# marvinli00/genie2

Measured on AMD Instinct MI355X. Metric: denoise-steps/sec (N=256, T=1000, batch=8), higher is better.
Workload: dtype f32 (pair-stack products as 3 f16 MFMAs on 2xf16-split operands, f32 accumulate); 1 GPU; unconditional N=256, T=1000, batch=8 per GPU, random-init base Denoiser (15.7M params), scale=0.6, reverse-loop steps 995..676; parallelism=replica per GPU x1, no data-path collective

## Files before the change

### genie2_amd/csrc/pair_hx_kernels.hip

```cpp
#include "hx_pair.h"


template <int NW>
__global__ __launch_bounds__(NW * 64, NW == 8 ? 1 : 2) void k_pair_transition_hx(
    float* __restrict__ z, const float* __restrict__ rmask, const unsigned char* __restrict__ wimg,
    const float* __restrict__ b1s, const float* __restrict__ b2s, int N, long long M, int n_hb, float sx, float c1, float c2, int rev) {
    extern __shared__ __attribute__((aligned(16))) unsigned char smb[];
    float* sb1 = reinterpret_cast<float*>(smb + 2 * HX_STAGE_BYTES);
    const int lane = threadIdx.x & 63, wave = UNI(threadIdx.x >> 6);
    const int h = lane >> 5, pl = lane & 31;
    const int n_wt = (int)((M + 31) / 32);
    const int n_tiles = (n_wt + NW - 1) / NW;
    const rsrc_t rw = hx_rsrc(wimg, (unsigned)(n_hb * HX_STAGE_BYTES));
    const rsrc_t rz = hx_rsrc(z, (unsigned)(M * 512));
    const rsrc_t rnull = hx_rsrc(z, 0u);
    const int lane16 = lane * 16;
    constexpr int PW = 32 / NW;
    auto issue = [&](int hb, int buf) {
#pragma unroll
        for (int q = 0; q < PW; ++q) {
            const int p = PW * wave + q;
            hx_dma(rw, smb + buf * HX_STAGE_BYTES + p * 1024, lane16, hb * HX_STAGE_BYTES + p * 1024);
        }
    };
// ... 334 lines not shown
    __syncthreads();
    int kc = 0;
    const int foff = (lane & 31) * CX_ROWB + (lane >> 5) * 16;
    for (int it = 0; it < total; ++it) {
        const bool last_chunk = kc == nk - 1;
        const int wn_next = last_chunk ? w + gridDim.x : w;
        const int kc_next = last_chunk ? 0 : kc + 1;
        if (it + 1 < total) gload(wn_next, kc_next);
        const unsigned char* sa = smb + (it & 1) * 4 * PLANE + foff;
        h8 ah[WT], al[WT], bh[WT], bl[WT];
#pragma unroll
        for (int m = 0; m < WT; ++m) {
            ah[m] = *reinterpret_cast<const h8*>(sa + (wm * WT + m) * 32 * CX_ROWB);
            al[m] = *reinterpret_cast<const h8*>(sa + PLANE + (wm * WT + m) * 32 * CX_ROWB);
        }
#pragma unroll
        for (int n = 0; n < WT; ++n) {
            bh[n] = *reinterpret_cast<const h8*>(sa + 2 * PLANE + (wn * WT + n) * 32 * CX_ROWB);
            bl[n] = *reinterpret_cast<const h8*>(sa + 3 * PLANE + (wn * WT + n) * 32 * CX_ROWB);
        }
#pragma unroll
        for (int m = 0; m < WT; ++m)
#pragma unroll
            for (int n = 0; n < WT; ++n) MFH3(ah[m], al[m], bh[n], bl[n], acc[m][n]);
        if (last_chunk) {
            int mi, i0, j0;
            decode(w, mi, i0, j0);
            if (mi < n_mat) {
                const int vst = ((4 * (lane >> 5)) * NP + (lane & 31)) * 4;
#pragma unroll
                for (int m = 0; m < WT; ++m)
#pragma unroll
                    for (int n = 0; n < WT; ++n) {
                        const int ib = i0 + (wm * WT + m) * 32, jb = j0 + (wn * WT + n) * 32;
                        if (ib < NP && jb < NP) {
                            const int sbase = ((mi * NP + ib) * NP + jb) * 4;
#pragma unroll
                            for (int r = 0; r < 16; ++r) {
                                const float v = acc[m][n][r] * cx;
                                hx_store(rx, v, vst, sbase + ((r & 3) + 8 * (r >> 2)) * NP * 4);
                            }
                        }
                        acc[m][n] = zero16();
                    }
            }
        }
        if (it + 1 < total) swrite((it + 1) & 1);
        __syncthreads();
        w = wn_next;
        kc = kc_next;
    }
}

#define CB_ROWB 80
#define CB_PLANE (256 * CB_ROWB)
__global__ __launch_bounds__(512, 1) void k_trimul_contract_hx_big(const unsigned* __restrict__ acm, const unsigned* __restrict__ bcm,
                                                                   float* __restrict__ xcm, int NP, int n_mat, unsigned cm_bytes, float cx, int rev) {
    extern __shared__ __attribute__((aligned(16))) unsigned char smb[];
    const int tid = threadIdx.x, lane = tid & 63;
    const int wave = UNI(tid >> 6);
    const int wm = wave >> 1, wn = wave & 1;
    const int nk = NP / 32;
    const rsrc_t ra = hx_rsrc(acm, cm_bytes), rb = hx_rsrc(bcm, cm_bytes), rx = hx_rsrc(xcm, cm_bytes);
    const int gq = tid >> 3, pc = tid & 7;
    const int lr = (gq & 0x38) | ((gq & 1) << 2) | ((gq >> 1) & 3);
    u32x4 rA[2][4], rB[2][4];
    auto mat_of = [&](int w) { return rev ? n_mat - 1 - w : w; };
    auto gload = [&](int w, int kc, auto set_tag) {
        constexpr int S = decltype(set_tag)::value;
        const int mbase = mat_of(w) * NP * NP * 4 + kc * 128;
#pragma unroll
        for (int u = 0; u < 4; ++u) {
            const int row = 64 * u + lr;
            const int vo = row < NP ? (row * NP * 4 + pc * 16) : 0x7FFFFFF0;
            rA[S][u] = __builtin_bit_cast(u32x4, __builtin_amdgcn_raw_buffer_load_b128(ra, vo, mbase, 0));
            rB[S][u] = __builtin_bit_cast(u32x4, __builtin_amdgcn_raw_buffer_load_b128(rb, vo, mbase, 0));
        }
    };
    auto swrite = [&](auto set_tag) {
        constexpr int S = decltype(set_tag)::value;
        unsigned char* sa = smb + lr * CB_ROWB + pc * 8;
#pragma unroll
        for (int u = 0; u < 4; ++u) {
            uint2 ahi, alo, bhi, blo;
            ahi.x = __builtin_amdgcn_perm(rA[S][u].y, rA[S][u].x, 0x05040100u); ahi.y = __builtin_amdgcn_perm(rA[S][u].w, rA[S][u].z, 0x05040100u);
            alo.x = __builtin_amdgcn_perm(rA[S][u].y, rA[S][u].x, 0x07060302u); alo.y = __builtin_amdgcn_perm(rA[S][u].w, rA[S][u].z, 0x07060302u);
            bhi.x = __builtin_amdgcn_perm(rB[S][u].y, rB[S][u].x, 0x05040100u); bhi.y = __builtin_amdgcn_perm(rB[S][u].w, rB[S][u].z, 0x05040100u);
            blo.x = __builtin_amdgcn_perm(rB[S][u].y, rB[S][u].x, 0x07060302u); blo.y = __builtin_amdgcn_perm(rB[S][u].w, rB[S][u].z, 0x07060302u);
            *reinterpret_cast<uint2*>(sa + 64 * u * CB_ROWB) = ahi;
            *reinterpret_cast<uint2*>(sa + CB_PLANE + 64 * u * CB_ROWB) = alo;
            *reinterpret_cast<uint2*>(sa + 2 * CB_PLANE + 64 * u * CB_ROWB) = bhi;
            *reinterpret_cast<uint2*>(sa + 3 * CB_PLANE + 64 * u * CB_ROWB) = blo;
        }
    };
    f32x16 acc[2][4];
#pragma unroll
    for (int m = 0; m < 2; ++m)
#pragma unroll
        for (int n = 0; n < 4; ++n) acc[m][n] = zero16();
    int w = blockIdx.x;
    if (w >= n_mat) return;
    const int my = (n_mat - 1 - w) / gridDim.x + 1;
    const int total = my * nk;
    int lw = w, lkc = 0, issued = 0;
    auto advance = [&]() { if (lkc == nk - 1) { lw += gridDim.x; lkc = 0; } else ++lkc; };
    gload(lw, lkc, std::integral_constant<int, 0>{}); advance(); ++issued;
    if (issued < total) { gload(lw, lkc, std::integral_constant<int, 1>{}); advance(); ++issued; }
    int kc = 0;
    const int foff = (lane & 31) * CB_ROWB + (lane >> 5) * 16;
    const bool wave_live = 64 * wm < NP && 128 * wn < NP;
    auto body = [&](int it, auto set_tag) {
        const bool last_chunk = kc == nk - 1;
        swrite(set_tag);
        __syncthreads();
        if (issued < total) { gload(lw, lkc, set_tag); advance(); ++issued; }
        if (wave_live) {
#pragma unroll
            for (int c = 0; c < 2; ++c) {
                const unsigned char* sa = smb + foff + c * 32;
                h8 ah[2], al[2], bh[4], bl[4];
#pragma unroll
                for (int m = 0; m < 2; ++m) {
                    ah[m] = *reinterpret_cast<const h8*>(sa + (wm * 2 + m) * 32 * CB_ROWB);
                    al[m] = *reinterpret_cast<const h8*>(sa + CB_PLANE + (wm * 2 + m) * 32 * CB_ROWB);
                }
#pragma unroll
                for (int n = 0; n < 4; ++n) {
                    bh[n] = *reinterpret_cast<const h8*>(sa + 2 * CB_PLANE + (wn * 4 + n) * 32 * CB_ROWB);
                    bl[n] = *reinterpret_cast<const h8*>(sa + 3 * CB_PLANE + (wn * 4 + n) * 32 * CB_ROWB);
                }
#pragma unroll
                for (int m = 0; m < 2; ++m)
#pragma unroll
                    for (int n = 0; n < 4; ++n) MFH3(ah[m], al[m], bh[n], bl[n], acc[m][n]);
            }
        }
        if (last_chunk) {
            const int mi = mat_of(w);
            const int vst = ((4 * (lane >> 5)) * NP + (lane & 31)) * 4;
#pragma unroll
            for (int m = 0; m < 2; ++m)
#pragma unroll
                for (int n = 0; n < 4; ++n) {
                    const int ib = (wm * 2 + m) * 32, jb = (wn * 4 + n) * 32;
                    if (ib < NP && jb < NP) {
                        const int sbase = ((mi * NP + ib) * NP + jb) * 4;
#pragma unroll
                        for (int r = 0; r < 16; ++r) {
                            const float v = acc[m][n][r] * cx;
#if HX_ABL & 512
                            if (r == 0)
#endif
                            hx_store(rx, v, vst, sbase + ((r & 3) + 8 * (r >> 2)) * NP * 4);
                        }
                    }
                    acc[m][n] = zero16();
                }
            w += gridDim.x;
            kc = 0;
        } else
            ++kc;
        __syncthreads();
    };
    for (int it = 0; it < total; it += 2) {
        body(it, std::integral_constant<int, 0>{});
        if (it + 1 < total) body(it + 1, std::integral_constant<int, 1>{});
    }
}

template <int NW>
__global__ __launch_bounds__(NW * 64, NW == 8 ? 1 : 2) void k_trimul_out_hx(
    float* __restrict__ z, const float* __restrict__ xcm, const unsigned char* __restrict__ wimg,
    const float* __restrict__ bgs, const float* __restrict__ bzs, int N, int NP, int n_wtiles, unsigned cm_bytes,
    unsigned z_bytes, float sx, float cg, float cz, int rev) {
    extern __shared__ __attribute__((aligned(16))) unsigned char smb[];
    const int lane = threadIdx.x & 63, wave = UNI(threadIdx.x >> 6);
    const int h = lane >> 5, pl = lane & 31;
    const int ntile = (N + 31) >> 5;
    const int n_tiles = (n_wtiles + NW - 1) / NW;
    const rsrc_t rw = hx_rsrc(wimg, 4 * HX_STAGE_BYTES);
    const rsrc_t rx = hx_rsrc(xcm, cm_bytes), rz = hx_rsrc(z, z_bytes);
    const int lane16 = lane * 16;
    constexpr int PW = 32 / NW;
    auto issue = [&](int s, int buf) {
#pragma unroll
        for (int q = 0; q < PW; ++q) {
            const int p = PW * wave + q;
            hx_dma(rw, smb + buf * HX_STAGE_BYTES + p * 1024, lane16, s * HX_STAGE_BYTES + p * 1024);
        }
    };
    unsigned char* zt = smb + 2 * HX_STAGE_BYTES + 2048 + wave * HX_ZT_BYTES;
    int tile = blockIdx.x;
    issue(0, 0);
    __syncthreads();
#pragma unroll 1
    for (; tile < n_tiles; tile += gridDim.x) {
        const int wt_raw = HX_PHYS(tile) * NW + wave;
        const bool act = wt_raw < n_wtiles;
        const int wt = act ? wt_raw : n_wtiles - 1;
        const int st = wt % ntile, i = (wt / ntile) % N, b = wt / (ntile * N);
        const int t0 = st * 32;
        const int nvalid = act ? min(32, N - t0) : 0;
        const int prow0 = (b * N + i) * N + t0;
        const bool more = tile + (int)gridDim.x < n_tiles;
        h8 zh[8], zl[8], xh[8], xl[8];
        {
            float4 raw[16], rawz[16];
            const int cs = NP * NP * 4;
            const int vx = (8 * h * NP * NP + pl) * 4;
            const int sxo = ((b * 128 * NP + i) * NP + t0) * 4;
#pragma unroll
            for (int kc = 0; kc < 8; ++kc) {
                raw[2 * kc].x = hx_load(rx, vx, sxo + (16 * kc + 0) * cs); raw[2 * kc].y = hx_load(rx, vx, sxo + (16 * kc + 1) * cs);
                raw[2 * kc].z = hx_load(rx, vx, sxo + (16 * kc + 2) * cs); raw[2 * kc].w = hx_load(rx, vx, sxo + (16 * kc + 3) * cs);
                raw[2 * kc + 1].x = hx_load(rx, vx, sxo + (16 * kc + 4) * cs); raw[2 * kc + 1].y = hx_load(rx, vx, sxo + (16 * kc + 5) * cs);
                raw[2 * kc + 1].z = hx_load(rx, vx, sxo + (16 * kc + 6) * cs); raw[2 * kc + 1].w = hx_load(rx, vx, sxo + (16 * kc + 7) * cs);
            }
            const int zsoff = prow0 * 512, znv = min(32, N - t0);
            hx_zt_dma(rz, zt, lane, zsoff, 512, znv, 0); hx_vm_done(); hx_zt_read(rawz, zt, pl, h, 0); hx_lds_done();
            hx_zt_dma(rz, zt, lane, zsoff, 512, znv, 1);
            hx_norm_split(xh, xl, raw, sx);
            hx_vm_done(); hx_zt_read(rawz, zt, pl, h, 1);
// ... 249 lines not shown
static int hx_nw() { return 8; }
static unsigned hx_grid(long long n_tiles, int nw, int cus) {
    const long long cap = (nw == 8 ? 1LL : 2LL) * cus;
    return (unsigned)(n_tiles < cap ? n_tiles : cap);
}

struct HxSlice { int b0, nb; hipStream_t st; int cus; unsigned launches; bool prof; };

static void pair_transition_slice(genie_ctx* h, HxSlice& v, const PairLayerW& w) {
    const int N = h->N;
    const long long M = (long long)v.nb * N * N;
    const long long n_wt = (M + 31) / 32;
    const int n_hb = h->d.pair_transition_n * 4;
    const HxTransW& x = w.hx_pt;
    hipLaunchKernelGGL(k_pair_transition_hx<8>, dim3(hx_grid((n_wt + 7) / 8, 8, v.cus)), dim3(512), HX_LDS_BYTES, v.st,
                       h->p + (size_t)v.b0 * N * N * 128, h->rmaskf + (size_t)v.b0 * N, x.img, x.b1s, x.b2s, N, M, n_hb, x.sx, x.c1, x.c2,
                       (int)(v.launches++ & 1));
}

struct HxTriGeom {
    int N, NP, ntile, nw, n_wt;
    unsigned *acm, *bcm; float* xcm; float* zs; const float* ms;
    unsigned cm_bytes, z_bytes;
};
static HxTriGeom tri_geom(genie_ctx* h, const HxSlice& v) {
    HxTriGeom g;
    g.N = h->N; g.NP = h->NP; g.ntile = (g.N + 31) / 32; g.nw = hx_nw();
    const size_t cm_off = (size_t)v.b0 * 128 * g.NP * g.NP;
    g.acm = reinterpret_cast<unsigned*>(h->acm) + cm_off;
    g.bcm = reinterpret_cast<unsigned*>(h->bcm) + cm_off;
    g.xcm = h->xcm + cm_off;
    g.n_wt = v.nb * g.N * g.ntile;
    g.cm_bytes = (unsigned)((size_t)v.nb * 128 * g.NP * g.NP * 4);
    g.z_bytes = (unsigned)((size_t)v.nb * g.N * g.N * 512);
    g.zs = h->p + (size_t)v.b0 * g.N * g.N * 128;
    g.ms = h->rmaskf + (size_t)v.b0 * g.N;
    return g;
}

static void trimul_proj_slice(genie_ctx* h, HxSlice& v, const TriMulW& w, bool outgoing) {
    const HxTriGeom g = tri_geom(h, v);
    const HxTriW& x = w.hx;
    hipStream_t st = v.st;
    ProfScope ps(h, st, KC_TRIMUL_PROJ, v.prof);
    const dim3 grid(hx_grid((g.n_wt + g.nw - 1) / g.nw, g.nw, v.cus)), block(g.nw * 64);
    const int rev = (int)(v.launches++ & 1);
#define HX_PROJ(OUT, NWV) hipLaunchKernelGGL((k_trimul_proj_hx<OUT, NWV>), grid, block, HX_LDS_BYTES, st, g.zs, g.ms, x.img_proj, \
                                         x.bias_proj, g.acm, g.bcm, g.N, g.NP, g.n_wt, g.cm_bytes, g.z_bytes, x.sx, x.cpa, x.cpb, x.cg, rev)
    if (outgoing) HX_PROJ(true, 8);
    else HX_PROJ(false, 8);
#undef HX_PROJ
}

static void trimul_contract_slice(genie_ctx* h, HxSlice& v, const TriMulW& w, bool transposed) {
    const HxTriGeom g = tri_geom(h, v);
    const HxTriW& x = w.hx;
    hipStream_t st = v.st;
    ProfScope ps(h, st, KC_TRIMUL_CONTRACT, v.prof);
    const int BC = v.nb * h->d.c_hidden_mul;
    const int ncu = v.cus;
    const int rev = (int)(v.launches++ & 1);
    const unsigned* pa = transposed ? g.bcm : g.acm;
    const unsigned* pb = transposed ? g.acm : g.bcm;
    if (g.NP > 192 && g.NP <= 256 && !getenv("GENIE_CONTRACT_TILED")) {
        hipLaunchKernelGGL(k_trimul_contract_hx_big, dim3(BC < ncu ? BC : ncu), dim3(512), 4 * CB_PLANE, st, pa, pb, g.xcm, g.NP, BC, g.cm_bytes,
                           x.cx, rev);
    } else if (g.NP >= 128) {
        const int tiles = (g.NP + 127) / 128;
        const int n_tiles = tiles * tiles * ((BC + 7) / 8) * 8;
        hipLaunchKernelGGL(k_trimul_contract_hx<2>, dim3(n_tiles < 3 * ncu ? n_tiles : 3 * ncu), dim3(256), 2 * 4 * 128 * CX_ROWB, st,
                           pa, pb, g.xcm, g.NP, BC, g.cm_bytes, x.cx, rev);
    } else {
        const int tiles = (g.NP + 63) / 64;
        const int n_tiles = tiles * tiles * ((BC + 7) / 8) * 8;
        hipLaunchKernelGGL(k_trimul_contract_hx<1>, dim3(n_tiles < 4 * ncu ? n_tiles : 4 * ncu), dim3(256), 2 * 4 * 64 * CX_ROWB, st,
                           pa, pb, g.xcm, g.NP, BC, g.cm_bytes, x.cx, rev);
    }
}

static void trimul_out_slice(genie_ctx* h, HxSlice& v, const TriMulW& w) {
    const HxTriGeom g = tri_geom(h, v);
    const HxTriW& x = w.hx;
    hipStream_t st = v.st;
    ProfScope ps(h, st, KC_TRIMUL_OUT, v.prof);
    const bool resident = getenv("GENIE_OUT_STREAMED") == nullptr;
    if (resident)
        hipLaunchKernelGGL(k_trimul_out_hx_r<8>, dim3(hx_grid((g.n_wt + 7) / 8, 8, v.cus)), dim3(512), 4 * HX_STAGE_BYTES, st, g.zs, g.xcm,
                           x.img_out, x.bgs, x.bzs, g.N, g.NP, g.n_wt, g.cm_bytes, g.z_bytes, x.sx, x.cgo, x.cz, (int)(v.launches++ & 1));
    else
        hipLaunchKernelGGL(k_trimul_out_hx<8>, dim3(hx_grid((g.n_wt + 7) / 8, 8, v.cus)), dim3(512), HX_LDS_BYTES, st, g.zs, g.xcm, x.img_out,
                           x.bgs, x.bzs, g.N, g.NP, g.n_wt, g.cm_bytes, g.z_bytes, x.sx, x.cgo, x.cz, (int)(v.launches++ & 1));
}

static void trimul_slice(genie_ctx* h, HxSlice& v, const TriMulW& w, bool outgoing) {
    trimul_proj_slice(h, v, w, outgoing);
    trimul_contract_slice(h, v, w, false);
    trimul_out_slice(h, v, w);
}

void launch_pair_fused(genie_ctx* h, hipStream_t st, const HxFusedW& f, const HxTriW& o, const HxTransW* t, const HxTriW* p, bool col);
bool launch_pair_stack_fused(genie_ctx* h, hipStream_t st, float* tap_trimul_out0, float* tap_layer0) {
    const int L = h->d.n_pair_transform_layer;
    if (!h->hx || L < 1 || getenv("GENIE_NO_PAIR_FUSE") || (getenv("GENIE_HX_SLICE") && atoi(getenv("GENIE_HX_SLICE")) > 0)) return false;
    if ((h->d.pair_transition_n * 4) & 1) return false;
    const size_t pbytes = (size_t)h->B * h->N * h->N * h->d.c_p * 4;
    HxSlice v{0, h->B, st, hx_num_cu(), h->hx_launches, h->prof};
    trimul_proj_slice(h, v, h->pair[0].out, true);
    for (int l = 0; l < L; ++l) {
        const PairLayerW& W = h->pair[l];
        trimul_contract_slice(h, v, W.out, true);
        h->hx_launches = v.launches;
        { ProfScope ps(h, st, KC_PAIR_FUSED_A); launch_pair_fused(h, st, W.fa, W.out.hx, nullptr, &W.in.hx, true); }
        v.launches = h->hx_launches;
        if (l == 0 && tap_trimul_out0) (void)hipMemcpyAsync(tap_trimul_out0, h->p, pbytes, hipMemcpyDeviceToDevice, st);
        trimul_contract_slice(h, v, W.in, false);
        if (l + 1 < L) {
            h->hx_launches = v.launches;
            { ProfScope ps(h, st, KC_PAIR_FUSED_B); launch_pair_fused(h, st, W.fb, W.in.hx, &W.hx_pt, &h->pair[l + 1].out.hx, false); }
            v.launches = h->hx_launches;
        } else {
            h->hx_launches = v.launches;
            { ProfScope ps(h, st, KC_PAIR_FUSED_B); launch_pair_fused(h, st, W.fb, W.in.hx, &W.hx_pt, nullptr, false); }
            v.launches = h->hx_launches;
        }
        if (l == 0 && tap_layer0) (void)hipMemcpyAsync(tap_layer0, h->p, pbytes, hipMemcpyDeviceToDevice, st);
    }
    h->hx_launches = v.launches;
    return true;
}

// ... 57 lines not shown
        const float sc = tiny ? 1.0f : __builtin_bit_cast(float, (unsigned)(268 - e) << 23);
        const float isc = (tiny ? 1.0f : __builtin_bit_cast(float, (unsigned)(e - 14) << 23)) * inv_sw;
        f32x16 acc[3];
#pragma unroll
        for (int blk = 0; blk < 3; ++blk)
#pragma unroll
            for (int r = 0; r < 16; ++r) acc[blk][r] = 0.f;
#pragma unroll
        for (int s = 0; s < 8; ++s) {
            const float xs[8] = {x[s][0].x, x[s][0].y, x[s][0].z, x[s][0].w, x[s][1].x, x[s][1].y, x[s][1].z, x[s][1].w};
            h8 bh, bl;
            hx_split8(xs, sc, bh, bl);
#pragma unroll
            for (int blk = 0; blk < 3; ++blk) {
                const h8 ah = hx_frag(ibw, blk * 8 + s, 0, lane), al = hx_frag(ibw, blk * 8 + s, 1, lane);
                MFH3(ah, al, bh, bl, acc[blk]);
            }
        }
        if (j0 + n < N) {
            const int b = bi / N, i = bi - b * N;
#pragma unroll
            for (int blk = 0; blk < 3; ++blk)
#pragma unroll
                for (int r = 0; r < 16; ++r) {
                    const int o = blk * 32 + (r & 3) + 8 * (r >> 2) + 4 * hf;
                    if (o < LH) out[((((size_t)o * B + b) * N + i) * N) + j0 + n] = fmaf(acc[blk][r], isc, sbias[o]);
                }
        }
    }
#pragma unroll
    for (int o = 32; o > 0; o >>= 1) amax = fmaxf(amax, __shfl_xor(amax, o));
    if (lane == 0 && __float_as_uint(amax) > *reinterpret_cast<volatile unsigned*>(pmax)) atomicMax(pmax, __float_as_uint(amax));
}

bool launch_ipa_bias_hx(genie_ctx* h, hipStream_t st) {
    const int LH = h->d.n_structure_layer * h->d.n_head_ipa;
    if (!h->hx || LH > 96 || h->d.c_p != 128 || getenv("GENIE_IPA_BIAS_F32")) return false;
    const HxGemmW* w = nullptr;
    for (int i = 0; i < h->n_hxg; ++i)
        if (h->hxg[i].w == h->ipa_bias_w) w = &h->hxg[i];
    if (!w) return false;
    const int N = h->N, n_tiles = h->B * N * ((N + 31) / 32);
    const int grid = n_tiles / 4 < 2 * hx_num_cu() ? (n_tiles + 3) / 4 : 2 * hx_num_cu();
    (void)hipMemsetAsync(h->pmax, 0, sizeof(unsigned), st);
    hipLaunchKernelGGL(k_ipa_bias_hx, dim3(grid), dim3(256), IB_UNITS * 2048 + 96 * 4, st, h->p, w->img, w->inv_s, h->ipa_bias_b, h->ipa_bias,
                       h->B, N, LH, n_tiles, (int)(h->hx_launches & 1), h->pmax);
    return true;
}

void pair_hx_kernels_init() {
#define HX_ATTR(k) (void)hipFuncSetAttribute(reinterpret_cast<const void*>(k), hipFuncAttributeMaxDynamicSharedMemorySize, HX_LDS_BYTES)
    HX_ATTR((k_trimul_proj_hx<true, 8>)); HX_ATTR((k_trimul_proj_hx<false, 8>));
    HX_ATTR(k_trimul_out_hx<8>); HX_ATTR(k_trimul_out_hx_r<8>);
    (void)hipFuncSetAttribute(reinterpret_cast<const void*>(k_trimul_contract_hx_big), hipFuncAttributeMaxDynamicSharedMemorySize, 4 * CB_PLANE);
#undef HX_ATTR
    (void)hipFuncSetAttribute(reinterpret_cast<const void*>(k_pair_transition_hx<8>), hipFuncAttributeMaxDynamicSharedMemorySize, HX_LDS_BYTES);
    (void)hipFuncSetAttribute(reinterpret_cast<const void*>(k_ipa_bias_hx), hipFuncAttributeMaxDynamicSharedMemorySize, IB_UNITS * 2048 + 96 * 4);
}
```

### genie2_amd/capi.py

```python
import ctypes as C
import os

import torch

_HERE = os.path.dirname(os.path.abspath(__file__))
LIB_PATH = os.environ.get('GENIE_HIP_LIB', os.path.join(_HERE, 'lib', 'libgenie_hip.so'))


class GenieDims(C.Structure):
    _fields_ = [
        ('c_s', C.c_int32), ('c_p', C.c_int32),
        ('c_pos_emb', C.c_int32), ('c_chain_emb', C.c_int32), ('c_timestep_emb', C.c_int32),
        ('relpos_k', C.c_int32),
        ('template_dist_n_bin', C.c_int32),
        ('template_dist_min', C.c_float), ('template_dist_step', C.c_float),
        ('n_pair_transform_layer', C.c_int32), ('c_hidden_mul', C.c_int32), ('pair_transition_n', C.c_int32),
        ('n_structure_layer', C.c_int32), ('n_structure_block', C.c_int32),
        ('c_hidden_ipa', C.c_int32), ('n_head_ipa', C.c_int32), ('n_qk_point', C.c_int32), ('n_v_point', C.c_int32),
        ('rescale', C.c_float),
        ('n_timestep', C.c_int32), ('max_n_res', C.c_int32), ('max_n_chain', C.c_int32),
    ]


class GenieFeatures(C.Structure):
# ... 5 lines not shown
class GenieTaps(C.Structure):
    _fields_ = [(k, C.c_void_p) for k in ('s', 'p', 's_final', 'rots_out', 'trans_out', 'p_init', 'p_layer0', 'states', 'p_trimul_out0',
                                              'ipa_cat0')]


class GenieGemmDesc(C.Structure):
    _fields_ = [(n, C.c_int32) for n in ('M', 'N', 'K', 'batch', 'nb2', 'nsplit', 'mode', 'terms', 'relu')] + \
               [(n, C.c_int64) for n in ('am', 'ak', 'bk', 'bn', 'cm', 'cn', 'a1', 'a2', 'b1', 'b2', 'c1', 'c2')] + [('alpha', C.c_float)] + \
               [('cblk', C.c_int32), ('cblk_m', C.c_int32), ('ctab', C.c_int64 * 8), ('atab', C.c_int64 * 8)]


class GenieTrainOpts(C.Structure):
    _fields_ = [('tri_dropout', C.c_float), ('ipa_dropout', C.c_float), ('transition_dropout', C.c_float), ('seed', C.c_uint32),
                ('train_mode', C.c_int32), ('fast_math', C.c_int32), ('struct_done_event', C.c_void_p)]


SYMBOLS = {
    'genie_create': (C.c_int, [C.POINTER(GenieDims), C.c_int, C.POINTER(C.c_void_p)]),
    'genie_destroy': (None, [C.c_void_p]),
    'genie_last_error': (C.c_char_p, [C.c_void_p]),
    'genie_weight_count': (C.c_size_t, [C.POINTER(GenieDims)]),
    'genie_load_weights': (C.c_int, [C.c_void_p, C.c_void_p, C.c_size_t]),
    'genie_set_tables': (C.c_int, [C.c_void_p, C.c_void_p, C.c_int, C.c_void_p, C.c_int, C.c_void_p, C.c_void_p]),
    'genie_prepare_features': (C.c_int, [C.c_void_p, C.c_void_p, C.c_int, C.c_int, C.POINTER(GenieFeatures)]),
    'genie_frenet': (C.c_int, [C.c_void_p, C.c_void_p, C.c_void_p, C.c_void_p]),
    'genie_frenet_frames': (C.c_int, [C.c_void_p, C.c_int, C.c_int, C.c_void_p, C.c_void_p, C.c_void_p, C.c_void_p]),
    'genie_denoise': (C.c_int, [C.c_void_p, C.c_void_p, C.c_void_p, C.c_void_p, C.c_void_p, C.c_void_p, C.c_void_p,
                                C.POINTER(GenieTaps)]),
    'genie_q_sample': (C.c_int, [C.c_void_p, C.c_void_p, C.c_void_p, C.c_void_p, C.c_void_p, C.c_void_p, C.c_void_p, C.c_void_p]),
    'genie_training_loss': (C.c_int, [C.c_void_p, C.c_void_p, C.c_void_p, C.c_void_p, C.c_float, C.c_void_p, C.c_void_p]),
    'genie_adam_step': (C.c_int, [C.c_void_p, C.c_size_t, C.c_void_p, C.c_void_p, C.c_void_p, C.c_void_p, C.c_double, C.c_double, C.c_double,
                                  C.c_double, C.c_int]),
    'genie_train_forward_backward': (C.c_int, [C.c_void_p, C.c_void_p, C.c_void_p, C.c_void_p, C.c_void_p, C.c_void_p, C.c_void_p, C.c_void_p,
                                                C.c_void_p, C.c_float, C.POINTER(GenieTrainOpts), C.c_void_p, C.c_void_p]),
    'genie_denoise_vjp': (C.c_int, [C.c_void_p] * 10),
    'genie_train_workspace_bytes': (C.c_size_t, [C.c_void_p]),
    'genie_train_kept_bytes': (C.c_size_t, [C.c_void_p]),
    'genie_train_gemm_flop': (C.c_double, [C.c_void_p]),
    'genie_train_gemm': (C.c_int, [C.c_void_p, C.POINTER(GenieGemmDesc), C.c_void_p, C.c_void_p, C.c_void_p, C.c_void_p, C.c_void_p, C.c_void_p]),
    'genie_p_sample': (C.c_int, [C.c_void_p, C.c_void_p, C.c_int, C.c_float, C.c_void_p, C.c_void_p, C.c_void_p,
                                 C.c_void_p]),
    'genie_sample_loop': (C.c_int, [C.c_void_p, C.c_void_p, C.c_float, C.c_void_p, C.c_void_p, C.c_int, C.c_int,
                                    C.c_void_p, C.c_void_p, C.c_void_p]),
    'genie_set_math': (C.c_int, [C.c_void_p, C.c_int]),
    'genie_get_math': (C.c_int, [C.c_void_p]),
    'genie_profile_enable': (C.c_int, [C.c_void_p, C.c_int]),
    'genie_profile_read': (C.c_int, [C.c_void_p, C.POINTER(C.c_char_p), C.POINTER(C.c_double),
                                     C.POINTER(C.c_int64), C.c_int]),
    'genie_probe_mfma': (C.c_int, [C.c_void_p, C.c_double, C.POINTER(C.c_double), C.POINTER(C.c_double)]),
    'genie_workspace_bytes': (C.c_size_t, [C.c_void_p]),
    'genie_motif_potential': (C.c_int, [C.c_void_p, C.c_int, C.c_int, C.c_void_p, C.c_int, C.c_int, C.c_int, C.c_void_p, C.c_void_p,
                                         C.c_void_p, C.c_void_p, C.c_void_p, C.c_void_p, C.c_void_p, C.c_size_t]),
    'genie_motif_potential_work_bytes': (C.c_size_t, [C.c_int, C.c_int]),
}

_lib = None


class GenieError(RuntimeError):
    pass


def load_library():
    global _lib
    if _lib is not None:
        return _lib
    if not os.path.exists(LIB_PATH):
        raise GenieError(
            f'{LIB_PATH} not found: build it with `python -m genie2_amd.build` '
            '(there is no CPU fallback for the denoising path)')
    lib = C.CDLL(LIB_PATH)
    for name, (res, args) in SYMBOLS.items():
        fn = getattr(lib, name)
        fn.restype = res
        fn.argtypes = args
    _lib = lib
    return lib


def check(handle, rc, what):
    if rc != 0:
        msg = load_library().genie_last_error(handle)
        raise GenieError(f'{what} failed (rc={rc}): {msg.decode() if msg else "?"}')
```

### include/genie_hip.h

```cpp
#ifndef GENIE_HIP_H
#define GENIE_HIP_H

#include <stddef.h>
#include <stdint.h>

#ifdef __cplusplus
extern "C" {
#endif

#define GENIE_OK            0
#define GENIE_E_ARG        -1
#define GENIE_E_STATE      -2
#define GENIE_E_HIP        -3
#define GENIE_E_NOMEM      -4

typedef struct genie_ctx* genie_handle_t;
typedef void* genie_stream_t;

typedef struct {
    int32_t c_s, c_p;
    int32_t c_pos_emb, c_chain_emb, c_timestep_emb;
    int32_t relpos_k;
    int32_t template_dist_n_bin;
    float   template_dist_min, template_dist_step;
// ... 7 lines not shown
typedef struct {
    const int32_t* aatype;
    const float*   atom_positions;
    const int32_t* residue_mask;
    const int32_t* residue_index;
    const int32_t* chain_index;
    const uint8_t* fixed_sequence_mask;
    const uint8_t* fixed_structure_mask;
    const uint8_t* interface_mask;
} genie_features_t;

typedef struct {
    float* s;
    float* p;
    float* s_final;
    float* rots_out;
    float* trans_out;
    float* p_init;
    float* p_layer0;
    float* states;
    float* p_trimul_out0;
    float* ipa_cat0;
} genie_taps_t;


int genie_create(const genie_dims_t* dims, int device, genie_handle_t* out);
void genie_destroy(genie_handle_t h);
const char* genie_last_error(genie_handle_t h);

size_t genie_weight_count(const genie_dims_t* dims);

int genie_load_weights(genie_handle_t h, const float* blob, size_t n_floats);

int genie_set_tables(genie_handle_t h, const float* pos_tab, int n_pos,
                     const float* chain_tab, int n_chain,
                     const float* t_tab, const float* sched);


int genie_prepare_features(genie_handle_t h, genie_stream_t stream, int B, int N,
                           const genie_features_t* feats);

int genie_frenet(genie_handle_t h, genie_stream_t stream, const float* trans ,
                 float* rots_out );

int genie_frenet_frames(genie_stream_t stream, int B, int N, const float* coords , const int32_t* chains,
                        const int32_t* mask, float* rots_out );

int genie_motif_potential(genie_stream_t stream, int B, int N, const float* x0 , int P, int S, int M,
                          const int32_t* seg_len , const int32_t* starts , const float* target ,
                          const float* var , float* logp_out , float* grad_out , void* work,
                          size_t work_bytes);
size_t genie_motif_potential_work_bytes(int B, int P);

int genie_denoise(genie_handle_t h, genie_stream_t stream,
                  const float* trans, const float* rots, const int32_t* timesteps,
                  const int8_t* quat_codes, float* z_out, const genie_taps_t* taps);

int genie_p_sample(genie_handle_t h, genie_stream_t stream, int step, float scale,
                   float* trans_inout, float* rots_out, const float* z, const float* eps);

int genie_sample_loop(genie_handle_t h, genie_stream_t stream, float scale,
                      const float* noise, const int8_t* quat_codes,
                      int first_step, int last_step,
                      float* trans_io, float* rots_io, float* record);


#define GENIE_MATH_F32 0
#define GENIE_MATH_HX 1
int genie_set_math(genie_handle_t h, int mode);
int genie_get_math(genie_handle_t h);


int genie_q_sample(genie_handle_t h, genie_stream_t stream, const float* x0 , const float* z ,
                   const float* c_x0 , const float* c_z , float* trans_out ,
                   float* rots_out );

int genie_training_loss(genie_handle_t h, genie_stream_t stream, const float* z_pred , const float* z ,
                        float condition_loss_weight, float* losses_out, float* grad_out);

int genie_adam_step(genie_stream_t stream, size_t n, float* p, const float* g, float* m, float* v, double lr, double beta1,
                    double beta2, double eps, int step);

typedef struct {
    float tri_dropout, ipa_dropout, transition_dropout;
    uint32_t seed;
    int32_t train_mode, fast_math;
    void* struct_done_event;
} genie_train_opts_t;
int genie_train_forward_backward(genie_handle_t h, genie_stream_t stream, const float* weights, float* grads, const float* trans ,
                                 const float* rots , const int32_t* timesteps , const float* z_target ,
                                 const int8_t* quat_codes , float condition_loss_weight, const genie_train_opts_t* opts,
                                 float* losses_out , float* z_pred_out);
int genie_denoise_vjp(genie_handle_t h, genie_stream_t stream, const float* weights, const float* trans, const float* rots,
                      const int32_t* timesteps, const int8_t* quat_codes, const float* dz, float* z_out, float* dtrans_out);
size_t genie_train_workspace_bytes(genie_handle_t h);
size_t genie_train_kept_bytes(genie_handle_t h);
double genie_train_gemm_flop(genie_handle_t h);

typedef struct {
    int32_t M, N, K, batch, nb2, nsplit, mode, terms, relu;
    int64_t am, ak, bk, bn, cm, cn, a1, a2, b1, b2, c1, c2;
    float alpha;
    int32_t cblk, cblk_m;
    int64_t ctab[8], atab[8];
} genie_gemm_desc_t;
int genie_train_gemm(genie_stream_t stream, const genie_gemm_desc_t* desc, const float* a, const float* b, float* c, const float* bias,
// ... 16 lines not shown
```

Baseline: 110.1 batch-steps/s.

## Add ring-buffered 5-stage contraction kernel for triangle-multiply at NP 193-256

Adds a new triangle-multiplication contraction kernel for padded sizes 193-256. It streams A and B k-chunks through a 5-slot LDS ring with direct-to-LDS DMA, keeping several pieces in flight, and writes the previous matrix's results while the next one's chunks load. It becomes the default path, replacing the staged big-plane kernel (still reachable through an env var). The goal is to hide global-load latency and barrier stalls between matrices, at the cost of 160KB of LDS per block and trickier waitcnt bookkeeping.

```diff
diff --git a/genie2_amd/csrc/pair_hx_kernels.hip b/genie2_amd/csrc/pair_hx_kernels.hip
--- a/genie2_amd/csrc/pair_hx_kernels.hip
+++ b/genie2_amd/csrc/pair_hx_kernels.hip
@@ -526,6 +526,116 @@
     }
 }
 
+#define CR_PIECE 32768
+#define CR_NS 5
+__global__ __launch_bounds__(512, 1) void k_trimul_contract_hx_ring(const unsigned* __restrict__ acm, const unsigned* __restrict__ bcm,
+                                                                    float* __restrict__ xcm, int NP, int n_mat, unsigned cm_bytes, float cx, int rev) {
+    extern __shared__ __attribute__((aligned(16))) unsigned char smb[];
+    const int tid = threadIdx.x, lane = tid & 63;
+    const int wave = UNI(tid >> 6);
+    const int wm = wave >> 1, wn = wave & 1;
+    const int nk = NP / 32;
+    const rsrc_t ra = hx_rsrc(acm, cm_bytes), rb = hx_rsrc(bcm, cm_bytes), rx = hx_rsrc(xcm, cm_bytes);
+    const int w0 = blockIdx.x;
+    if (w0 >= n_mat) return;
+    const int total = ((n_mat - 1 - w0) / gridDim.x + 1) * nk;
+    const int n_pieces = 2 * total;
+    auto mat_of = [&](int t) { const int w = w0 + t * (int)gridDim.x; return rev ? n_mat - 1 - w : w; };
+    int dvo[4];
+#pragma unroll
+    for (int q = 0; q < 4; ++q) {
+        const int row = 32 * wave + 8 * q + (lane >> 3);
+        dvo[q] = row < NP ? row * NP * 4 + (((lane & 7) ^ ((row >> 1) & 7)) << 4) : 0x7FFFFFF0;
+    }
+    auto issue = [&](int p) {
+        const int g = p >> 1, t = g / nk, kc = g - t * nk;
+        const int soff = mat_of(t) * NP * NP * 4 + kc * 128;
+        unsigned char* dst = smb + (p % CR_NS) * CR_PIECE + wave * 4096;
+        const rsrc_t r = (p & 1) ? rb : ra;
+#pragma unroll
+        for (int q = 0; q < 4; ++q) hx_dma(r, dst + q * 1024, dvo[q], soff);
+    };
+    const int fr = lane & 31, fh = lane >> 5, swz = (fr >> 1) & 7;
+    const int g0[2] = {((2 * fh) ^ swz) << 4, ((4 + 2 * fh) ^ swz) << 4};
+    const int g1[2] = {((2 * fh + 1) ^ swz) << 4, ((4 + 2 * fh + 1) ^ swz) << 4};
+    auto frag = [&](const unsigned char* piece, int blk, int c, h8& hi, h8& lo) {
+        const unsigned char* rowp = piece + (32 * blk + fr) * 128;
+        const u32x4 x0 = *reinterpret_cast<const u32x4*>(rowp + g0[c]);
+        const u32x4 x1 = *reinterpret_cast<const u32x4*>(rowp + g1[c]);
+        u32x4 vh, vl;
+        vh.x = __builtin_amdgcn_perm(x0.y, x0.x, 0x05040100u); vl.x = __builtin_amdgcn_perm(x0.y, x0.x, 0x07060302u);
+        vh.y = __builtin_amdgcn_perm(x0.w, x0.z, 0x05040100u); vl.y = __builtin_amdgcn_perm(x0.w, x0.z, 0x07060302u);
+        vh.z = __builtin_amdgcn_perm(x1.y, x1.x, 0x05040100u); vl.z = __builtin_amdgcn_perm(x1.y, x1.x, 0x07060302u);
+        vh.w = __builtin_amdgcn_perm(x1.w, x1.z, 0x05040100u); vl.w = __builtin_amdgcn_perm(x1.w, x1.z, 0x07060302u);
+        hi = __builtin_bit_cast(h8, vh);
+        lo = __builtin_bit_cast(h8, vl);
+    };
+    f32x16 acc[2][4];
+#pragma unroll
+    for (int m = 0; m < 2; ++m)
+#pragma unroll
+        for (int n = 0; n < 4; ++n) acc[m][n] = zero16();
+    const int vst = ((4 * fh) * NP + fr) * 4;
+    auto store_block = [&](int mi, int m, int n) {
+        const int ib = (wm * 2 + m) * 32, jb = (wn * 4 + n) * 32;
+        const int vo = (ib < NP && jb < NP) ? vst : 0x7FFFFFF0;
+        const int sbase = ((mi * NP + ib) * NP + jb) * 4;
+#pragma unroll
+        for (int r = 0; r < 16; ++r) hx_store(rx, acc[m][n][r] * cx, vo, sbase + ((r & 3) + 8 * (r >> 2)) * NP * 4);
+    };
+    auto chunk = [&](const unsigned char* pa, const unsigned char* pb) {
+#pragma unroll
+        for (int c = 0; c < 2; ++c) {
+            PIPE_FENCE();
+            h8 ah[2], al[2], bh[4], bl[4];
+#pragma unroll
+            for (int m = 0; m < 2; ++m) frag(pa, wm * 2 + m, c, ah[m], al[m]);
+#pragma unroll
+            for (int n = 0; n < 4; ++n) frag(pb, wn * 4 + n, c, bh[n], bl[n]);
+#pragma unroll
+            for (int m = 0; m < 2; ++m)
+#pragma unroll
+                for (int n = 0; n < 4; ++n) {
+                    MFH3(ah[m], al[m], bh[n], bl[n], acc[m][n]);
+                }
+        }
+    };
+    issue(0); issue(1); issue(2);
+    int t = 0, kc = 0;
+    bool stored = false;
+#pragma unroll 1
+    for (int g = 0; g < total; ++g) {
+        if (stored) asm volatile("s_waitcnt vmcnt(63)" ::: "memory");
+        else if (g + 1 < total) asm volatile("s_waitcnt vmcnt(4)" ::: "memory");
+        else asm volatile("s_waitcnt vmcnt(0)" ::: "memory");
+        asm volatile("s_waitcnt lgkmcnt(0)" ::: "memory");
+        hx_stage_barrier();
+        if (2 * g + 3 < n_pieces) issue(2 * g + 3);
+        if (2 * g + 4 < n_pieces) issue(2 * g + 4);
+        const unsigned char* pa = smb + ((2 * g) % CR_NS) * CR_PIECE;
+        const unsigned char* pb = smb + ((2 * g + 1) % CR_NS) * CR_PIECE;
+        stored = kc == 0 && t > 0;
+        if (stored) {
+            const int mi = mat_of(t - 1);
+#pragma unroll
+            for (int m = 0; m < 2; ++m)
+#pragma unroll
+                for (int n = 0; n < 4; ++n) {
+                    store_block(mi, m, n);
+                    acc[m][n] = zero16();
+                }
+        }
+        chunk(pa, pb);
+        if (++kc == nk) { kc = 0; ++t; }
+        PIPE_FENCE();
+    }
+    const int mi = mat_of(t - 1);
+#pragma unroll
+    for (int m = 0; m < 2; ++m)
+#pragma unroll
+        for (int n = 0; n < 4; ++n) store_block(mi, m, n);
+}
+
 template <int NW>
 __global__ __launch_bounds__(NW * 64, NW == 8 ? 1 : 2) void k_trimul_out_hx(
     float* __restrict__ z, const float* __restrict__ xcm, const unsigned char* __restrict__ wimg,
@@ -892,8 +1002,12 @@
     const unsigned* pa = transposed ? g.bcm : g.acm;
     const unsigned* pb = transposed ? g.acm : g.bcm;
     if (g.NP > 192 && g.NP <= 256 && !getenv("GENIE_CONTRACT_TILED")) {
-        hipLaunchKernelGGL(k_trimul_contract_hx_big, dim3(BC < ncu ? BC : ncu), dim3(512), 4 * CB_PLANE, st, pa, pb, g.xcm, g.NP, BC, g.cm_bytes,
-                           x.cx, rev);
+        if (getenv("GENIE_CONTRACT_STAGED"))
+            hipLaunchKernelGGL(k_trimul_contract_hx_big, dim3(BC < ncu ? BC : ncu), dim3(512), 4 * CB_PLANE, st, pa, pb, g.xcm, g.NP, BC,
+                               g.cm_bytes, x.cx, rev);
+        else
+            hipLaunchKernelGGL(k_trimul_contract_hx_ring, dim3(BC < ncu ? BC : ncu), dim3(512), CR_NS * CR_PIECE, st, pa, pb, g.xcm, g.NP,
+                               BC, g.cm_bytes, x.cx, rev);
     } else if (g.NP >= 128) {
         const int tiles = (g.NP + 127) / 128;
         const int n_tiles = tiles * tiles * ((BC + 7) / 8) * 8;
@@ -1069,6 +1183,8 @@
     HX_ATTR((k_trimul_proj_hx<true, 8>)); HX_ATTR((k_trimul_proj_hx<false, 8>));
     HX_ATTR(k_trimul_out_hx<8>); HX_ATTR(k_trimul_out_hx_r<8>);
     (void)hipFuncSetAttribute(reinterpret_cast<const void*>(k_trimul_contract_hx_big), hipFuncAttributeMaxDynamicSharedMemorySize, 4 * CB_PLANE);
+    (void)hipFuncSetAttribute(reinterpret_cast<const void*>(k_trimul_contract_hx_ring), hipFuncAttributeMaxDynamicSharedMemorySize,
+                              CR_NS * CR_PIECE);
 #undef HX_ATTR
     (void)hipFuncSetAttribute(reinterpret_cast<const void*>(k_pair_transition_hx<8>), hipFuncAttributeMaxDynamicSharedMemorySize, HX_LDS_BYTES);
     (void)hipFuncSetAttribute(reinterpret_cast<const void*>(k_ipa_bias_hx), hipFuncAttributeMaxDynamicSharedMemorySize, IB_UNITS * 2048 + 96 * 4);
```

Result: no change. 110.4 batch-steps/s (median of 6 runs) (+0.3%).

## Stream trimul contraction operands via async DMA ring into swizzled LDS

Applied to the files above, without the earlier changes.

Rewrites the big-N triangle-multiplication contraction kernel so operand chunks are loaded by direct global-to-LDS DMA into a 5-slot ring of 32KB pieces, with a swizzled layout. The f16 hi/lo split now happens at fragment-read time instead of register staging and an LDS write-back. vmcnt waits replace the double register-set prefetch and one of the two barriers per step. The aim is to overlap global loads with MFMA work and cut register pressure and LDS write traffic, at the cost of extra permute work on every fragment read. It also adds optional timestamp instrumentation and a standalone C entry point for the contraction.

```diff
diff --git a/genie2_amd/capi.py b/genie2_amd/capi.py
--- a/genie2_amd/capi.py
+++ b/genie2_amd/capi.py
@@ -81,6 +81,7 @@
     'genie_motif_potential': (C.c_int, [C.c_void_p, C.c_int, C.c_int, C.c_void_p, C.c_int, C.c_int, C.c_int, C.c_void_p, C.c_void_p,
                                          C.c_void_p, C.c_void_p, C.c_void_p, C.c_void_p, C.c_void_p, C.c_size_t]),
     'genie_motif_potential_work_bytes': (C.c_size_t, [C.c_int, C.c_int]),
+    'genie_hx_contract': (C.c_int, [C.c_void_p, C.c_int, C.c_int, C.c_void_p, C.c_void_p, C.c_void_p, C.c_float, C.c_int]),
 }
 
 _lib = None
diff --git a/genie2_amd/csrc/pair_hx_kernels.hip b/genie2_amd/csrc/pair_hx_kernels.hip
--- a/genie2_amd/csrc/pair_hx_kernels.hip
+++ b/genie2_amd/csrc/pair_hx_kernels.hip
@@ -410,8 +410,25 @@
     }
 }
 
-#define CB_ROWB 80
-#define CB_PLANE (256 * CB_ROWB)
+#define CB_PIECE 32768
+#define CB_RING 5
+#define CB_LDS_BYTES (CB_RING * CB_PIECE)
+#if HX_ABL & 128
+#define CB_TS_STEPS 64
+__device__ __attribute__((aligned(16))) unsigned long long g_cb_ts[256][8][CB_TS_STEPS * 6];
+extern "C" int genie_cb_debug_read(unsigned long long* out) {
+    return (int)hipMemcpyFromSymbol(out, HIP_SYMBOL(g_cb_ts), sizeof(g_cb_ts));
+}
+#define CB_NTS 3
+#define CB_STAMP(i) tsv[i] = __builtin_amdgcn_s_memtime()
+#else
+#define CB_NTS 0
+#define CB_STAMP(i) do { } while (0)
+#endif
+template <int N> __device__ __forceinline__ void cb_vm_wait() {
+    static_assert(N >= 0 && N < 64, "vmcnt");
+    __builtin_amdgcn_s_waitcnt((N & 15) | ((N >> 4) << 14) | (7 << 4) | (15 << 8));
+}
 __global__ __launch_bounds__(512, 1) void k_trimul_contract_hx_big(const unsigned* __restrict__ acm, const unsigned* __restrict__ bcm,
                                                                    float* __restrict__ xcm, int NP, int n_mat, unsigned cm_bytes, float cx, int rev) {
     extern __shared__ __attribute__((aligned(16))) unsigned char smb[];
@@ -420,80 +437,96 @@
     const int wm = wave >> 1, wn = wave & 1;
     const int nk = NP / 32;
     const rsrc_t ra = hx_rsrc(acm, cm_bytes), rb = hx_rsrc(bcm, cm_bytes), rx = hx_rsrc(xcm, cm_bytes);
-    const int gq = tid >> 3, pc = tid & 7;
-    const int lr = (gq & 0x38) | ((gq & 1) << 2) | ((gq >> 1) & 3);
-    u32x4 rA[2][4], rB[2][4];
-    auto mat_of = [&](int w) { return rev ? n_mat - 1 - w : w; };
-    auto gload = [&](int w, int kc, auto set_tag) {
-        constexpr int S = decltype(set_tag)::value;
-        const int mbase = mat_of(w) * NP * NP * 4 + kc * 128;
-#pragma unroll
-        for (int u = 0; u < 4; ++u) {
-            const int row = 64 * u + lr;
-            const int vo = row < NP ? (row * NP * 4 + pc * 16) : 0x7FFFFFF0;
-            rA[S][u] = __builtin_bit_cast(u32x4, __builtin_amdgcn_raw_buffer_load_b128(ra, vo, mbase, 0));
-            rB[S][u] = __builtin_bit_cast(u32x4, __builtin_amdgcn_raw_buffer_load_b128(rb, vo, mbase, 0));
+    int w = blockIdx.x;
+    if (w >= n_mat) return;
+    const int total = ((n_mat - 1 - w) / (int)gridDim.x + 1) * nk;
+    const int n_pieces = 2 * total;
+    auto mat_of = [&](int m) { return rev ? n_mat - 1 - m : m; };
+    int dvo[4];
+#pragma unroll
+    for (int j = 0; j < 4; ++j) {
+        const int row = 32 * wave + 8 * j + (lane >> 3);
+        dvo[j] = min(row, NP - 1) * NP * 4 + (((lane & 7) ^ ((row >> 1) & 7)) << 4);
+    }
+    int iw = w, ikc = 0, iop = 0;
+    auto issue = [&](int p) {
+        unsigned char* dst = smb + (p % CB_RING) * CB_PIECE + wave * 4096;
+        const int soff = mat_of(iw) * NP * NP * 4 + ikc * 128;
+        if (iop) {
+#pragma unroll
+            for (int j = 0; j < 4; ++j) hx_dma(rb, dst + j * 1024, dvo[j], soff);
+            iop = 0;
+            if (++ikc == nk) { ikc = 0; iw += gridDim.x; }
+        } else {
+#pragma unroll
+            for (int j = 0; j < 4; ++j) hx_dma(ra, dst + j * 1024, dvo[j], soff);
+            iop = 1;
         }
     };
-    auto swrite = [&](auto set_tag) {
-        constexpr int S = decltype(set_tag)::value;
-        unsigned char* sa = smb + lr * CB_ROWB + pc * 8;
-#pragma unroll
-        for (int u = 0; u < 4; ++u) {
-            uint2 ahi, alo, bhi, blo;
-            ahi.x = __builtin_amdgcn_perm(rA[S][u].y, rA[S][u].x, 0x05040100u); ahi.y = __builtin_amdgcn_perm(rA[S][u].w, rA[S][u].z, 0x05040100u);
-            alo.x = __builtin_amdgcn_perm(rA[S][u].y, rA[S][u].x, 0x07060302u); alo.y = __builtin_amdgcn_perm(rA[S][u].w, rA[S][u].z, 0x07060302u);
-            bhi.x = __builtin_amdgcn_perm(rB[S][u].y, rB[S][u].x, 0x05040100u); bhi.y = __builtin_amdgcn_perm(rB[S][u].w, rB[S][u].z, 0x05040100u);
-            blo.x = __builtin_amdgcn_perm(rB[S][u].y, rB[S][u].x, 0x07060302u); blo.y = __builtin_amdgcn_perm(rB[S][u].w, rB[S][u].z, 0x07060302u);
-            *reinterpret_cast<uint2*>(sa + 64 * u * CB_ROWB) = ahi;
-            *reinterpret_cast<uint2*>(sa + CB_PLANE + 64 * u * CB_ROWB) = alo;
-            *reinterpret_cast<uint2*>(sa + 2 * CB_PLANE + 64 * u * CB_ROWB) = bhi;
-            *reinterpret_cast<uint2*>(sa + 3 * CB_PLANE + 64 * u * CB_ROWB) = blo;
-        }
+    const int sw = (lane >> 1) & 7, h = lane >> 5;
+    const int frow = (lane & 31) * 128;
+    auto frag = [&](const unsigned char* piece, int blk, int c, h8& hi, h8& lo) {
+        const unsigned char* r = piece + blk * 32 * 128 + frow;
+        const u32x4 p = *reinterpret_cast<const u32x4*>(r + (((4 * c + 2 * h) ^ sw) << 4));
+        const u32x4 q = *reinterpret_cast<const u32x4*>(r + (((4 * c + 2 * h + 1) ^ sw) << 4));
+        u32x4 H, L;
+        H.x = __builtin_amdgcn_perm(p.y, p.x, 0x05040100u); L.x = __builtin_amdgcn_perm(p.y, p.x, 0x07060302u);
+        H.y = __builtin_amdgcn_perm(p.w, p.z, 0x05040100u); L.y = __builtin_amdgcn_perm(p.w, p.z, 0x07060302u);
+        H.z = __builtin_amdgcn_perm(q.y, q.x, 0x05040100u); L.z = __builtin_amdgcn_perm(q.y, q.x, 0x07060302u);
+        H.w = __builtin_amdgcn_perm(q.w, q.z, 0x05040100u); L.w = __builtin_amdgcn_perm(q.w, q.z, 0x07060302u);
+        hi = __builtin_bit_cast(h8, H);
+        lo = __builtin_bit_cast(h8, L);
     };
     f32x16 acc[2][4];
 #pragma unroll
     for (int m = 0; m < 2; ++m)
 #pragma unroll
         for (int n = 0; n < 4; ++n) acc[m][n] = zero16();
-    int w = blockIdx.x;
-    if (w >= n_mat) return;
-    const int my = (n_mat - 1 - w) / gridDim.x + 1;
-    const int total = my * nk;
-    int lw = w, lkc = 0, issued = 0;
-    auto advance = [&]() { if (lkc == nk - 1) { lw += gridDim.x; lkc = 0; } else ++lkc; };
-    gload(lw, lkc, std::integral_constant<int, 0>{}); advance(); ++issued;
-    if (issued < total) { gload(lw, lkc, std::integral_constant<int, 1>{}); advance(); ++issued; }
+#if HX_ABL & 128
+    unsigned long long tsv[6] = {0, 0, 0, 0, 0, 0}, tsp[6] = {0, 0, 0, 0, 0, 0};
+    unsigned long long* ts_p = g_cb_ts[blockIdx.x & 255][wave];
+#endif
+    for (int p = 0; p < 3 && p < n_pieces; ++p) issue(p);
+    const bool wave_live = 64 * wm < NP && 128 * wn < NP;
     int kc = 0;
-    const int foff = (lane & 31) * CB_ROWB + (lane >> 5) * 16;
-    const bool wave_live = 64 * wm < NP && 128 * wn < NP;
-    auto body = [&](int it, auto set_tag) {
-        const bool last_chunk = kc == nk - 1;
-        swrite(set_tag);
-        __syncthreads();
-        if (issued < total) { gload(lw, lkc, set_tag); advance(); ++issued; }
+    for (int t = 0; t < total; ++t) {
+        CB_STAMP(0);
+        if (t > 0 && kc == 0) cb_vm_wait<63>();
+        else if (t + 1 < total) { if (t > 0) cb_vm_wait<4 + CB_NTS>(); else cb_vm_wait<4>(); }
+        else { if (t > 0) cb_vm_wait<CB_NTS>(); else cb_vm_wait<0>(); }
+        CB_STAMP(1);
+        hx_lds_done();
+        hx_stage_barrier();
+        CB_STAMP(2);
+        if (2 * t + 3 < n_pieces) issue(2 * t + 3);
+        if (2 * t + 4 < n_pieces) issue(2 * t + 4);
+#if HX_ABL & 128
+        {
+            unsigned long long* d = ts_p + 6 * (t > 0 && t <= CB_TS_STEPS ? t - 1 : CB_TS_STEPS - 1);
+#pragma unroll
+            for (int i = 0; i < 3; ++i)
+                if (lane == 0) *reinterpret_cast<u32x4*>(d + 2 * i) = __builtin_bit_cast(u32x4, (unsigned long long __attribute__((ext_vector_type(2)))){tsp[2 * i], tsp[2 * i + 1]});
+        }
+#endif
+        CB_STAMP(3);
         if (wave_live) {
+            const unsigned char* pa = smb + ((2 * t) % CB_RING) * CB_PIECE;
+            const unsigned char* pb = smb + ((2 * t + 1) % CB_RING) * CB_PIECE;
 #pragma unroll
             for (int c = 0; c < 2; ++c) {
-                const unsigned char* sa = smb + foff + c * 32;
                 h8 ah[2], al[2], bh[4], bl[4];
 #pragma unroll
-                for (int m = 0; m < 2; ++m) {
-                    ah[m] = *reinterpret_cast<const h8*>(sa + (wm * 2 + m) * 32 * CB_ROWB);
-                    al[m] = *reinterpret_cast<const h8*>(sa + CB_PLANE + (wm * 2 + m) * 32 * CB_ROWB);
-                }
-#pragma unroll
-                for (int n = 0; n < 4; ++n) {
-                    bh[n] = *reinterpret_cast<const h8*>(sa + 2 * CB_PLANE + (wn * 4 + n) * 32 * CB_ROWB);
-                    bl[n] = *reinterpret_cast<const h8*>(sa + 3 * CB_PLANE + (wn * 4 + n) * 32 * CB_ROWB);
-                }
+                for (int m = 0; m < 2; ++m) frag(pa, wm * 2 + m, c, ah[m], al[m]);
+#pragma unroll
+                for (int n = 0; n < 4; ++n) frag(pb, wn * 4 + n, c, bh[n], bl[n]);
 #pragma unroll
                 for (int m = 0; m < 2; ++m)
 #pragma unroll
                     for (int n = 0; n < 4; ++n) MFH3(ah[m], al[m], bh[n], bl[n], acc[m][n]);
             }
         }
-        if (last_chunk) {
+        CB_STAMP(4);
+        if (kc == nk - 1) {
             const int mi = mat_of(w);
             const int vst = ((4 * (lane >> 5)) * NP + (lane & 31)) * 4;
 #pragma unroll
@@ -506,9 +539,6 @@
 #pragma unroll
                         for (int r = 0; r < 16; ++r) {
                             const float v = acc[m][n][r] * cx;
-#if HX_ABL & 512
-                            if (r == 0)
-#endif
                             hx_store(rx, v, vst, sbase + ((r & 3) + 8 * (r >> 2)) * NP * 4);
                         }
                     }
@@ -518,11 +548,11 @@
             kc = 0;
         } else
             ++kc;
-        __syncthreads();
-    };
-    for (int it = 0; it < total; it += 2) {
-        body(it, std::integral_constant<int, 0>{});
-        if (it + 1 < total) body(it + 1, std::integral_constant<int, 1>{});
+        CB_STAMP(5);
+#if HX_ABL & 128
+#pragma unroll
+        for (int i = 0; i < 6; ++i) tsp[i] = tsv[i];
+#endif
     }
 }
 
@@ -881,30 +911,30 @@
 #undef HX_PROJ
 }
 
+static void hx_contract_launch(hipStream_t st, const unsigned* pa, const unsigned* pb, float* xcm, int NP, int n_mat, unsigned cm_bytes,
+                               float cx, int rev, int ncu) {
+    if (NP > 192 && NP <= 256 && !getenv("GENIE_CONTRACT_TILED")) {
+        hipLaunchKernelGGL(k_trimul_contract_hx_big, dim3(n_mat < ncu ? n_mat : ncu), dim3(512), CB_LDS_BYTES, st, pa, pb, xcm, NP, n_mat,
+                           cm_bytes, cx, rev);
+    } else if (NP >= 128) {
+        const int tiles = (NP + 127) / 128;
+        const int n_tiles = tiles * tiles * ((n_mat + 7) / 8) * 8;
+        hipLaunchKernelGGL(k_trimul_contract_hx<2>, dim3(n_tiles < 3 * ncu ? n_tiles : 3 * ncu), dim3(256), 2 * 4 * 128 * CX_ROWB, st,
+                           pa, pb, xcm, NP, n_mat, cm_bytes, cx, rev);
+    } else {
+        const int tiles = (NP + 63) / 64;
+        const int n_tiles = tiles * tiles * ((n_mat + 7) / 8) * 8;
+        hipLaunchKernelGGL(k_trimul_contract_hx<1>, dim3(n_tiles < 4 * ncu ? n_tiles : 4 * ncu), dim3(256), 2 * 4 * 64 * CX_ROWB, st,
+                           pa, pb, xcm, NP, n_mat, cm_bytes, cx, rev);
+    }
+}
+
 static void trimul_contract_slice(genie_ctx* h, HxSlice& v, const TriMulW& w, bool transposed) {
     const HxTriGeom g = tri_geom(h, v);
-    const HxTriW& x = w.hx;
-    hipStream_t st = v.st;
-    ProfScope ps(h, st, KC_TRIMUL_CONTRACT, v.prof);
-    const int BC = v.nb * h->d.c_hidden_mul;
-    const int ncu = v.cus;
+    ProfScope ps(h, v.st, KC_TRIMUL_CONTRACT, v.prof);
     const int rev = (int)(v.launches++ & 1);
-    const unsigned* pa = transposed ? g.bcm : g.acm;
-    const unsigned* pb = transposed ? g.acm : g.bcm;
-    if (g.NP > 192 && g.NP <= 256 && !getenv("GENIE_CONTRACT_TILED")) {
-        hipLaunchKernelGGL(k_trimul_contract_hx_big, dim3(BC < ncu ? BC : ncu), dim3(512), 4 * CB_PLANE, st, pa, pb, g.xcm, g.NP, BC, g.cm_bytes,
-                           x.cx, rev);
-    } else if (g.NP >= 128) {
-        const int tiles = (g.NP + 127) / 128;
-        const int n_tiles = tiles * tiles * ((BC + 7) / 8) * 8;
-        hipLaunchKernelGGL(k_trimul_contract_hx<2>, dim3(n_tiles < 3 * ncu ? n_tiles : 3 * ncu), dim3(256), 2 * 4 * 128 * CX_ROWB, st,
-                           pa, pb, g.xcm, g.NP, BC, g.cm_bytes, x.cx, rev);
-    } else {
-        const int tiles = (g.NP + 63) / 64;
-        const int n_tiles = tiles * tiles * ((BC + 7) / 8) * 8;
-        hipLaunchKernelGGL(k_trimul_contract_hx<1>, dim3(n_tiles < 4 * ncu ? n_tiles : 4 * ncu), dim3(256), 2 * 4 * 64 * CX_ROWB, st,
-                           pa, pb, g.xcm, g.NP, BC, g.cm_bytes, x.cx, rev);
-    }
+    hx_contract_launch(v.st, transposed ? g.bcm : g.acm, transposed ? g.acm : g.bcm, g.xcm, g.NP, v.nb * h->d.c_hidden_mul, g.cm_bytes,
+                       w.hx.cx, rev, v.cus);
 }
 
 static void trimul_out_slice(genie_ctx* h, HxSlice& v, const TriMulW& w) {
@@ -1068,8 +1098,19 @@
 #define HX_ATTR(k) (void)hipFuncSetAttribute(reinterpret_cast<const void*>(k), hipFuncAttributeMaxDynamicSharedMemorySize, HX_LDS_BYTES)
     HX_ATTR((k_trimul_proj_hx<true, 8>)); HX_ATTR((k_trimul_proj_hx<false, 8>));
     HX_ATTR(k_trimul_out_hx<8>); HX_ATTR(k_trimul_out_hx_r<8>);
-    (void)hipFuncSetAttribute(reinterpret_cast<const void*>(k_trimul_contract_hx_big), hipFuncAttributeMaxDynamicSharedMemorySize, 4 * CB_PLANE);
+    (void)hipFuncSetAttribute(reinterpret_cast<const void*>(k_trimul_contract_hx_big), hipFuncAttributeMaxDynamicSharedMemorySize, CB_LDS_BYTES);
 #undef HX_ATTR
     (void)hipFuncSetAttribute(reinterpret_cast<const void*>(k_pair_transition_hx<8>), hipFuncAttributeMaxDynamicSharedMemorySize, HX_LDS_BYTES);
     (void)hipFuncSetAttribute(reinterpret_cast<const void*>(k_ipa_bias_hx), hipFuncAttributeMaxDynamicSharedMemorySize, IB_UNITS * 2048 + 96 * 4);
 }
+
+void pair_kernels_init();
+extern "C" int genie_hx_contract(genie_stream_t stream, int n_mat, int N, const unsigned* a, const unsigned* b, float* x, float cx,
+                                 int rev) {
+    const int NP = (N + 31) / 32 * 32;
+    if (!a || !b || !x || n_mat < 1 || N < 1 || NP > 256 || (size_t)n_mat * NP * NP * 4 > 0xFFFFFFFFu) return GENIE_E_ARG;
+    static const bool inited = (pair_kernels_init(), true);
+    (void)inited;
+    hx_contract_launch((hipStream_t)stream, a, b, x, NP, n_mat, (unsigned)((size_t)n_mat * NP * NP * 4), cx, rev ? 1 : 0, hx_num_cu());
+    return hipGetLastError() == hipSuccess ? 0 : GENIE_E_ARG;
+}
diff --git a/include/genie_hip.h b/include/genie_hip.h
--- a/include/genie_hip.h
+++ b/include/genie_hip.h
@@ -83,6 +83,8 @@
                           size_t work_bytes);
 size_t genie_motif_potential_work_bytes(int B, int P);
 
+int genie_hx_contract(genie_stream_t stream, int n_mat, int N, const unsigned* a, const unsigned* b, float* x, float cx, int rev);
+
 int genie_denoise(genie_handle_t h, genie_stream_t stream,
                   const float* trans, const float* rots, const int32_t* timesteps,
                   const int8_t* quat_codes, float* z_out, const genie_taps_t* taps);
```

New measurement: 106.6 batch-steps/s before, 106.9 batch-steps/s after (median of 6 runs). No clear change (+0.2%).
